# ZhangXiaze/DeepPointMap

Hardware: AMD Instinct MI355X
Metric: LiDAR frames/s (encode+match+register), 65 536 pts/frame (higher is better)
Workload: dtype f32 (attention scores K Q^T and P V, Linear / Conv1d (+ LayerNorm) layers with K <= 2048 as exact three-way bf16 splits: 6 bf16 products per fp32 product, fp32 accumulate -- fp32 accuracy, bf16 matrix pipe; all else fp32); 1 GPU; synthetic 64x65536-pt scans per GPU: Encoder.forward + consecutive-frame registration_forward (256x256) + information matrix per frame; points_per_frame=65536, parallelism=frame-sharded x1, one RCCL gather of descriptors+edges per step, weights=procedural (deeppointmap_amd/weights.py), allocator_reserve_gib=16, geometry_waits_for_caller_stream=True

## Files before the change

deeppointmap_amd/_lib.py:

```python
from __future__ import annotations

import ctypes
import os

import torch
from ctypes import c_char_p, c_double, c_int, c_longlong, c_size_t, c_uint, c_void_p

_HERE = os.path.dirname(os.path.abspath(__file__))
LIB_PATH = os.environ.get("DPM_LIB") or os.path.join(_HERE, "libdpm_hip.so")
VERSION_EXPERIMENT = 0x40000000

P, I, D, LL = c_void_p, c_int, c_double, c_longlong

SIGNATURES = {
    "dpm_version": (I, []),
    "dpm_error_string": (c_char_p, [I]),
    "dpm_prepare_points": (I, [P, P, I, I, I, P, P, P]),
    "dpm_to_channel_first": (I, [P, I, I, I, P, P]),
    "dpm_to_channel_first_ld": (I, [P, I, I, I, P, I, P]),
    "dpm_emit_descriptors": (I, [P, P, P, I, I, I, D, P, P, P, P, P]),
    "dpm_nested_levels": (I, [P, P, I, I, I, P, P, P, P, P]),
    "dpm_gather_frames": (I, [P, LL, I, I, I, P, I, P, P]),
    "dpm_fps_workspace_bytes": (c_size_t, [I, I, I]),
    "dpm_fps": (I, [P, P, I, I, I, P, P, P, P, P]),
# ... 44 lines not shown
    "dpm_match_workspace_bytes": (c_size_t, [I, I, I, I]),
    "dpm_match_topk": (I, [P, P, I, I, I, I, D, I, P, P, P, P]),
    "dpm_pairing_workspace_bytes": (c_size_t, [I, I, I]),
    "dpm_dual_softmax_topk": (I, [P, I, I, I, D, I, P, P, P, P]),
    "dpm_gather_pairs": (I, [P, P, P, I, I, I, I, I, P, P, P, P]),
    "dpm_mean_rows": (I, [P, I, I, I, P, I, P]),
    "dpm_kabsch_workspace_bytes": (c_size_t, [I, I]),
    "dpm_corr_kabsch": (I, [P, P, I, LL, P, I, LL, P, P, P, I, I, D, I, D, P, P, P, I, P]),
    "dpm_preprocess_workspace_bytes": (c_size_t, [LL]),
    "dpm_preprocess_scan": (I, [P, I, I, D, D, D, D, LL, P, P, I, P, P, P]),
    "dpm_knn_self_workspace_bytes": (c_size_t, [I]),
    "dpm_knn_self": (I, [P, I, I, D, P, P, P, P, P]),
    "dpm_point_normals": (I, [P, I, D, P, P, P]),
    "dpm_lowpass_similarity": (I, [P, P, I, I, I, P, P]),
    "dpm_stat_filter": (I, [P, I, D, I, D, P, P, P, P, P, P]),
    "dpm_filter_dc_workspace_bytes": (c_size_t, [I, I]),
    "dpm_outlier_filter_dc": (I, [P, P, P, I, I, D, D, D, P, P, P, P, P]),
    "dpm_lowpass_filter_dc": (I, [P, P, P, I, D, I, D, I, D, D, P, P, P, P, P]),
    "dpm_augment_workspace_bytes": (c_size_t, [I, LL]),
    "dpm_ground_filter": (I, [P, P, P, I, I, I, D, D, I, P, P, P, P, P]),
    "dpm_voxel_select": (I, [P, P, P, I, D, I, LL, P, P, P, P, P]),
    "dpm_mask_select": (I, [P, P, P, I, I, D, D, P, D, P, I, P, P, P, P, P]),
    "dpm_points_affine": (I, [P, P, I, I, P, P, P]),
    "dpm_points_deskew": (I, [P, P, P, I, I, P, I, I, P, D, P]),
    "dpm_gather_points": (I, [P, P, P, I, P, I, I, P, P, P, P]),
    "dpm_pack_frames": (I, [P, P, P, I, I, P, P, P, P]),
    "dpm_ingest_frames": (I, [P, P, LL, I, I, I, P, P, P, P, P]),
    "dpm_map_tile": (I, [P, P, P, P, I, I, I, P, P]),
    "dpm_infomat_workspace_bytes": (c_size_t, [I, I, I]),
    "dpm_information_matrix": (I, [P, I, P, I, P, D, P, P, P]),
    "dpm_information_matrix_batched": (I, [P, I, P, P, I, P, I, D, P, I, P, P]),
    "dpm_infomat_build_grids": (I, [P, I, P, I, D, P, P]),
    "dpm_infomat_search_grids": (I, [P, I, P, P, I, P, I, D, P, I, P, P]),
    "dpm_icp_workspace_bytes": (c_size_t, [I, I]),
    "dpm_icp_refine_batched": (I, [P, I, I, P, P, P, P, I, P, I, P, P, I, D, D, P, P, P, P, P, P, P, P, P]),
    "dpm_voxel_map_workspace_bytes": (c_size_t, [LL]),
    "dpm_voxel_map_init": (I, [LL, P, P]),
    "dpm_voxel_map_bounds": (I, [P, P, P, I, LL, P, P]),
    "dpm_voxel_map_insert": (I, [P, P, P, I, LL, LL, LL, D, D, D, D, P, P]),
    "dpm_voxel_map_finish": (I, [LL, P, P]),
    "dpm_voxel_map_emit": (I, [P, LL, D, D, D, D, P, P, I, P]),
    "dpm_reg_loss_pairs": (I, [P, P, I, I, I, D, P, P, P, P, P]),
    "dpm_reg_loss_workspace_bytes": (c_size_t, [I, I, I, I]),
    "dpm_reg_loss_forward": (I, [P, P, P, P, P, P, P, P, I, I, I, I, D, D, I, P, P, P, P, P, P]),
    "dpm_reg_loss_backward": (I, [P, P, P, P, I, I, I, I, D, D, I, P, P, P, P, P, P]),
    "dpm_attention_train_workspace_bytes": (c_size_t, [I, I, I, I]),
    "dpm_attention_train_forward": (I, [P, I, LL, P, I, LL, P, I, LL, P, I, LL, P, I, I, I, I, I, P, P]),
    "dpm_attention_train_backward": (I, [P, I, LL, P, I, LL, P, I, LL, P, I, LL, P, P, I, LL, P, P, P, P, I, I, I, I, I, P, P]),
    "dpm_offset_pairs_count": (I, [P, P, P, P, I, I, I, D, P, P, P]),
    "dpm_offset_pairs_fill": (I, [P, P, P, P, I, I, I, D, P, P, P]),
    "dpm_offset_pairs_gather": (I, [P, I, P, I, I, LL, I, P, P]),
    "dpm_offset_pairs_segment_sum": (I, [P, I, P, P, LL, I, P, P]),
    "dpm_group_train_forward": (I, [P, P, P, P, P, I, P, P, I, I, I, I, I, D, P, P, P]),
    "dpm_group_train_workspace_bytes": (c_size_t, [I, I, I, I, I]),
    "dpm_group_train_backward": (I, [P, P, P, P, P, I, P, I, I, I, I, I, D, P, P, P, P, P, P, P, P]),
    "dpm_loop_pool_workspace_bytes": (c_size_t, [I, I, I]),
    "dpm_loop_pool_forward": (I, [P, I, P, P, I, I, I, P, P, P]),
    "dpm_loop_pool_backward": (I, [P, I, P, P, P, I, I, I, P, P, P, P]),
    "dpm_loop_bce_forward": (I, [P, P, I, P, P, P, P]),
    "dpm_dense_train_workspace_bytes": (c_size_t, [LL, I, I]),
    "dpm_dense_train_forward": (I, [P, I, P, I, P, P, P, P, P, LL, I, I, I, P, P, P, P]),
    "dpm_dense_train_backward_rows": (I, [P, P, P, P, P, LL, I, I, P, P, P, P, P, P]),
    "dpm_dense_train_backward_gemm": (I, [P, P, I, P, I, LL, I, I, P, P, P, P, P]),
    "dpm_map_poses": (I, [P, P, P, P, P, I, I, I, P, P, P]),
    "dpm_map_assemble_fwd": (I, [P, P, P, P, P, I, I, I, I, I, D, P, P, P, P, P, P, P]),
    "dpm_map_assemble_bwd": (I, [P, P, I, I, I, I, I, P, P]),
# ... 93 lines not shown
```

deeppointmap_amd/csrc/infomat.hip:

```cpp
#include "block_scan.h"
#include "cell_grid.h"
#include "workspace.h"
#include <type_traits>

namespace {

constexpr int GMAX = 512;

struct PairArgs {
    const float *pcd1, *pcd2;
    const int32_t *f1, *f2;
    long long stride1, stride2;
    const float *Rt;
    int rt_stride;
    float *out;
    int out_stride;
    char *ws;
    size_t ws_stride;
    int N1, N2;
};

struct GridHdr {
    float lox, loy, inv_cs;
    int gx, gy, ncell;
    int H;
    int qexp;
};

__device__ __forceinline__ const float *pair_p1(const PairArgs &a, int p) {
    return a.pcd1 + (size_t)(a.f1 ? a.f1[p] : p) * a.stride1;
}
__device__ __forceinline__ const float *pair_p2(const PairArgs &a, int p) {
    return a.pcd2 + (size_t)(a.f2 ? a.f2[p] : p) * a.stride2;
}
__device__ __forceinline__ GridHdr *pair_hdr(const PairArgs &a, int p) { return (GridHdr *)(a.ws + (size_t)p * a.ws_stride); }
__device__ __forceinline__ int *pair_count(const PairArgs &a, int p) { return (int *)(a.ws + (size_t)p * a.ws_stride + 256); }
__device__ __forceinline__ float4 *pair_sorted(const PairArgs &a, int p) {
    return (float4 *)(a.ws + (size_t)p * a.ws_stride + 256 + sizeof(int) * (size_t)(GMAX * GMAX + 1) + 12);
}
__device__ __forceinline__ long long *pair_partial(const PairArgs &a, int p) {
    return (long long *)(pair_sorted(a, p) + a.N2);
}

constexpr int GB_CHUNK = 4096;

__device__ __forceinline__ float *pair_bounds(const PairArgs &a, int p);

__global__ __launch_bounds__(256) void grid_bounds_kernel(PairArgs A) {
    const int chunk = blockIdx.x, pair = blockIdx.y, chunks = gridDim.x;
    const float *p2 = pair_p2(A, pair);
    const int N2 = A.N2;
    __shared__ float red[5][4];
    const int t = threadIdx.x, lane = t & 63, w = t >> 6;
    float lox = __builtin_inff(), loy = lox, hix = -lox, hiy = -lox, amax = 0.f;
    constexpr int PPT = GB_CHUNK / 256;
    const int i0 = chunk * GB_CHUNK + t;
    float xs[PPT], ys[PPT], zs[PPT];
#pragma unroll
    for (int u = 0; u < PPT; ++u) {
        const int i = min(i0 + u * 256, N2 - 1);
        xs[u] = p2[i], ys[u] = p2[(size_t)N2 + i], zs[u] = p2[2 * (size_t)N2 + i];
    }
#pragma unroll
    for (int u = 0; u < PPT; ++u) {
        lox = fminf(lox, xs[u]), hix = fmaxf(hix, xs[u]), loy = fminf(loy, ys[u]), hiy = fmaxf(hiy, ys[u]);
        amax = fmaxf(amax, fmaxf(fmaxf(fabsf(xs[u]), fabsf(ys[u])), fabsf(zs[u])));
    }
#pragma unroll
    for (int off = 32; off > 0; off >>= 1) {
        lox = fminf(lox, __shfl_xor(lox, off, 64)), loy = fminf(loy, __shfl_xor(loy, off, 64));
        hix = fmaxf(hix, __shfl_xor(hix, off, 64)), hiy = fmaxf(hiy, __shfl_xor(hiy, off, 64));
        amax = fmaxf(amax, __shfl_xor(amax, off, 64));
// ... 144 lines not shown
#pragma unroll
    for (int u = 0; u < RB; ++u)
        if (lo + lane + u * 64 < hi) atomicAdd(&c[cell_coord(v[u].x, lox, inv_cs, gx)], 1);
    for (int p = lo + lane + RB * 64; p < hi; p += 64) atomicAdd(&c[cell_coord(tmp[p].x, lox, inv_cs, gx)], 1);
    __builtin_amdgcn_wave_barrier();
    const int per = (gx + 63) / 64, a = min(lane * per, gx), b = min(a + per, gx);
    int sum = 0;
    for (int k = a; k < b; ++k) sum += c[k];
    int run = lo + wave_scan_inclusive(sum) - sum;
    for (int k = a; k < b; ++k) {
        const int n = c[k];
        c[k] = run, run += n;
    }
    __builtin_amdgcn_wave_barrier();
    for (int k = lane; k < gx; k += 64) start[(size_t)row * gx + k] = c[k];
    if (row == gy - 1 && lane == 0) start[(size_t)gy * gx] = A.N2;
    __builtin_amdgcn_wave_barrier();
#pragma unroll
    for (int u = 0; u < RB; ++u)
        if (lo + lane + u * 64 < hi) sorted[atomicAdd(&c[cell_coord(v[u].x, lox, inv_cs, gx)], 1)] = v[u];
    for (int p = lo + lane + RB * 64; p < hi; p += 64) {
        const float4 q = tmp[p];
        sorted[atomicAdd(&c[cell_coord(q.x, lox, inv_cs, gx)], 1)] = q;
    }
}

__device__ __forceinline__ float quad_xor1(float v) { return __int_as_float(dpp_i<0xB1, 0xF>(__float_as_int(v))); }
__device__ __forceinline__ float quad_xor2(float v) { return __int_as_float(dpp_i<0x4E, 0xF>(__float_as_int(v))); }
__device__ __forceinline__ float quad_min(float v) {
    v = fminf(v, quad_xor1(v));
    return fminf(v, quad_xor2(v));
}

__global__ __launch_bounds__(256) void nn1_match_kernel(PairArgs A, float r2, int ordered) {
    int pair, blk;
    pair_block(blk, pair);
    const float *p1 = pair_p1(A, pair);
    const float *p2 = pair_p2(A, pair);
    const int N1 = A.N1, N2 = A.N2;
    const float *Rt = A.Rt + (size_t)pair * A.rt_stride;
    const GridHdr *hdr = pair_hdr(A, pair);
    const int *start = pair_count(A, pair);
    const float4 *sorted = pair_sorted(A, pair);
    __shared__ int s_qp;
    __shared__ long long sred[4][10];
    const int quad = threadIdx.x >> 2, ql = threadIdx.x & 3;
    if (threadIdx.x == 0) s_qp = -1;
    __syncthreads();
    if (ordered && A.f1 && A.f2 && N1 == N2)
        for (int t = threadIdx.x; t < (int)gridDim.y; t += 256)
            if (A.f2[t] == A.f1[pair]) atomicMax(&s_qp, t);
    __syncthreads();
    const float4 *qsorted = s_qp >= 0 ? pair_sorted(A, s_qp) : nullptr;
    const int gx = hdr->gx, gy = hdr->gy, H = hdr->H;
    const float inv_cs = hdr->inv_cs, cs = 1.0f / inv_cs, lox = hdr->lox, loy = hdr->loy;
    const float k2 = cs * cs * (1.f - 1e-5f);
    constexpr int NR = 5;
    int win[4] = {-1, -1, -1, -1};
    const int i_own = blk * 256 + ql * 64 + quad;
    float o_qx, o_qy, o_qz, o_below, o_above;
    int o_rlo[NR], o_rhi[NR];
    {
        const int ic = min(i_own, N1 - 1);
        float x, y, z;
        if (qsorted) {
            const float4 q4 = qsorted[ic];
            x = q4.x, y = q4.y, z = q4.z;
        } else {
            x = p1[ic], y = p1[(size_t)N1 + ic], z = p1[2 * (size_t)N1 + ic];
        }
        o_qx = fmaf(Rt[2], z, fmaf(Rt[1], y, Rt[0] * x)) + Rt[9];
        o_qy = fmaf(Rt[5], z, fmaf(Rt[4], y, Rt[3] * x)) + Rt[10];
        o_qz = fmaf(Rt[8], z, fmaf(Rt[7], y, Rt[6] * x)) + Rt[11];
        const float fx = (o_qx - lox) * inv_cs, fy = (o_qy - loy) * inv_cs;
        const float flx = floorf(fx), fly = floorf(fy);
        const int cx = (int)fmaxf(fminf(flx, 1e6f), -1e6f), cy = (int)fmaxf(fminf(fly, 1e6f), -1e6f);
        const int xa = min(max(cx - H, 0), gx), xb = min(max(cx + H + 1, 0), gx);
#pragma unroll
        for (int r = 0; r < NR; ++r) {
            const int k = (r + 1) / 2 * ((r & 1) ? -1 : 1);
            const int yy = cy + k;
            const bool in = yy >= 0 && yy < gy && (r < 3 || H > 1);
            const int yc = min(max(yy, 0), gy - 1);
            o_rlo[r] = in ? start[yc * gx + xa] : 0, o_rhi[r] = in ? start[yc * gx + xb] : 0;
        }
        o_below = fy - fly, o_above = fly + 1.f - fy;
    }
    auto one_query = [&](auto Jc) {
        constexpr int j = decltype(Jc)::value;
        constexpr int BC = j * 0x55;
        const int i = blk * 256 + j * 64 + quad;
        if (i >= N1) return;
        auto from_j = [&](int v) { return __builtin_amdgcn_update_dpp(v, v, BC, 0xF, 0xF, false); };
        auto from_jf = [&](float v) { return __int_as_float(from_j(__float_as_int(v))); };
        const float qx = from_jf(o_qx), qy = from_jf(o_qy), qz = from_jf(o_qz);
        int rlo[NR], rhi[NR];
#pragma unroll
        for (int r = 0; r < NR; ++r) rlo[r] = from_j(o_rlo[r]), rhi[r] = from_j(o_rhi[r]);
        const float mg = 1e-3f;
        unsigned long long best = ~0ull;
        auto offer = [&](const float4 t, bool ok) {
            const float dx = qx - t.x, dy = qy - t.y, dz = qz - t.z;
            const float d = (dx * dx + dy * dy) + dz * dz;
            const unsigned long long key = ((unsigned long long)__float_as_uint(d) << 32) | (unsigned)__float_as_int(t.w);
            best = (ok && key < best) ? key : best;
        };
        auto rest = [&](int from, int hi) {
            for (int p = from; p < hi; p += 8) {
                const float4 t0 = sorted[p], t1 = sorted[min(p + 4, hi - 1)];
                offer(t0, true), offer(t1, p + 4 < hi);
            }
        };
        {
            float4 t[3][2];
            bool ok[3][2];
#pragma unroll
            for (int r = 0; r < 3; ++r) {
#pragma unroll
                for (int u = 0; u < 2; ++u) {
                    const int p = rlo[r] + ql + 4 * u;
                    ok[r][u] = p < rhi[r];
                    t[r][u] = sorted[ok[r][u] ? p : 0];
                }
            }
#pragma unroll
            for (int r = 0; r < 3; ++r) offer(t[r][0], ok[r][0]), offer(t[r][1], ok[r][1]);
#pragma unroll
            for (int r = 0; r < 3; ++r) rest(rlo[r] + ql + 8, rhi[r]);
        }
        if (H > 1) {
            const float bd = best == ~0ull ? r2 : fminf(__uint_as_float((unsigned)(best >> 32)), r2);
            const float below = from_jf(o_below), above = from_jf(o_above);
            const float g0 = fmaxf(below + 1.f - mg, 0.f), g1 = fmaxf(above + 1.f - mg, 0.f);
            const int h3 = (g0 * g0 * k2 > bd) ? 0 : rhi[3], h4 = (g1 * g1 * k2 > bd) ? 0 : rhi[4];
            const int p3 = rlo[3] + ql, p4 = rlo[4] + ql;
            const float4 a0 = sorted[p3 < h3 ? p3 : 0], a1 = sorted[p3 + 4 < h3 ? p3 + 4 : 0];
            const float4 b0 = sorted[p4 < h4 ? p4 : 0], b1 = sorted[p4 + 4 < h4 ? p4 + 4 : 0];
            offer(a0, p3 < h3), offer(a1, p3 + 4 < h3), offer(b0, p4 < h4), offer(b1, p4 + 4 < h4);
            rest(p3 + 8, h3), rest(p4 + 8, h4);
        }
#pragma unroll
        for (int step = 0; step < 2; ++step) {
            const float blo = __int_as_float((int)(unsigned)best), bhi = __int_as_float((int)(unsigned)(best >> 32));
            const unsigned olo = (unsigned)__float_as_int(step ? quad_xor2(blo) : quad_xor1(blo));
            const unsigned ohi = (unsigned)__float_as_int(step ? quad_xor2(bhi) : quad_xor1(bhi));
            const unsigned long long o = ((unsigned long long)ohi << 32) | olo;
            best = o < best ? o : best;
        }
        win[j] = (best != ~0ull && __uint_as_float((unsigned)(best >> 32)) <= r2) ? (int)(unsigned)best : -1;
    };
    one_query(std::integral_constant<int, 0>{});
    one_query(std::integral_constant<int, 1>{});
    one_query(std::integral_constant<int, 2>{});
    one_query(std::integral_constant<int, 3>{});
    long long m[10] = {0, 0, 0, 0, 0, 0, 0, 0, 0, 0};
    if (ql == 0) {
        const float qs = ldexpf(1.f, hdr->qexp);
        float X[4], Y[4], Z[4];
#pragma unroll
        for (int j = 0; j < 4; ++j) {
            const int oi = max(win[j], 0);
            X[j] = p2[oi], Y[j] = p2[(size_t)N2 + oi], Z[j] = p2[2 * (size_t)N2 + oi];
        }
#pragma unroll
        for (int j = 0; j < 4; ++j) {
            if (win[j] < 0) continue;
            const long long x = (long long)__float2int_rn(X[j] * qs), y = (long long)__float2int_rn(Y[j] * qs),
                            z = (long long)__float2int_rn(Z[j] * qs);
            m[0] += 1, m[1] += x, m[2] += y, m[3] += z, m[4] += x * x, m[5] += y * y, m[6] += z * z;
            m[7] += x * y, m[8] += x * z, m[9] += y * z;
        }
    }
    const int lane = threadIdx.x & 63, w = threadIdx.x >> 6;
#pragma unroll
    for (int k = 0; k < 10; ++k) {
        long long v = m[k];
#pragma unroll
        for (int off = 32; off > 0; off >>= 1) v += __shfl_xor(v, off, 64);
        if (lane == 0) sred[w][k] = v;
    }
    __syncthreads();
    if (threadIdx.x < 10)
        pair_partial(A, pair)[(size_t)blk * 10 + threadIdx.x] =
            (sred[0][threadIdx.x] + sred[1][threadIdx.x]) + (sred[2][threadIdx.x] + sred[3][threadIdx.x]);
}

__global__ __launch_bounds__(64) void infomat_finalize_kernel(PairArgs A) {
    const long long *part = pair_partial(A, blockIdx.x);
    const int nblk = (A.N1 + 255) / 256, lane = threadIdx.x;
    __shared__ long long s[10];
    for (int k = 0; k < 10; ++k) {
        long long v = 0;
        for (int b = lane; b < nblk; b += 64) v += part[(size_t)b * 10 + k];
        v = wave_sum(v);
        if (lane == 0) s[k] = v;
    }
    __syncthreads();
    if (lane != 0) return;
    float *out = A.out + (size_t)blockIdx.x * A.out_stride;
    const int qexp = pair_hdr(A, blockIdx.x)->qexp;
    const double u = ldexp(1.0, -qexp), u2 = ldexp(1.0, -2 * qexp);
    const double n = (double)s[0], x = (double)s[1] * u, y = (double)s[2] * u, z = (double)s[3] * u, xx = (double)s[4] * u2,
                 yy = (double)s[5] * u2, zz = (double)s[6] * u2, xy = (double)s[7] * u2, xz = (double)s[8] * u2,
                 yz = (double)s[9] * u2;
    const double G[36] = {zz + yy, -xy,     -xz,     0,  -z, y,
                          -xy,     zz + xx, -yz,     z,  0,  -x,
                          -xz,     -yz,     yy + xx, -y, x,  0,
                          0,       z,       -y,      n,  0,  0,
                          -z,      0,       x,       0,  n,  0,
                          y,       -x,      0,       0,  0,  n};
    for (int i = 0; i < 36; ++i) out[i] = (float)G[i];
}

}

static size_t ws_slice_bytes(int N1, int N2) {
    size_t b = 256 + sizeof(int) * (size_t)(GMAX * GMAX + 1) + 12 + sizeof(float4) * (size_t)N2 +
               10 * sizeof(long long) * (size_t)dpm_cdiv(N1, 256) +
               sizeof(float4) * (size_t)N2 + sizeof(int) * ((size_t)dpm_cdiv(N2, GB_CHUNK) * (GMAX + 8) + GMAX + 4);
    return ws_align256(b);
}

extern "C" size_t dpm_infomat_workspace_bytes(int n_pairs, int N1, int N2) {
    return 256 + (size_t)n_pairs * ws_slice_bytes(N1, N2);
}

static int launch_grid(PairArgs A, int n_pairs, double radius, hipStream_t st) {
    const int fine = dpm_knob("DPM_NN1_FINE", 1);
    const int chunks = dpm_cdiv(A.N2, GB_CHUNK);
    hipLaunchKernelGGL(grid_bounds_kernel, dim3(chunks, n_pairs), dim3(256), 0, st, A);
    hipLaunchKernelGGL(grid_setup_kernel, dim3(n_pairs), dim3(64), 0, st, A, (float)radius, fine, chunks);
    if (dpm_knob("DPM_ABLATE_GRID", 0)) return dpm_launch_status();
    hipLaunchKernelGGL(grid_rows_kernel<false>, dim3(chunks, n_pairs), dim3(256), 0, st, A);
    hipLaunchKernelGGL(grid_offsets_kernel, dim3(n_pairs), dim3(256), 0, st, A);
    hipLaunchKernelGGL(grid_rows_kernel<true>, dim3(chunks, n_pairs), dim3(256), 0, st, A);
    hipLaunchKernelGGL(grid_cells_kernel, dim3(GMAX / 4, n_pairs), dim3(256), 0, st, A);
    return dpm_launch_status();
}

static int launch_search(PairArgs A, int n_pairs, double radius, hipStream_t st) {
    if (dpm_knob("DPM_ABLATE_NN1", 0)) return DPM_OK;
    const int ord = dpm_knob("DPM_NN1_ORDERED", 1);
    hipLaunchKernelGGL(nn1_match_kernel, dim3(dpm_cdiv(A.N1, 256), n_pairs), dim3(256), 0, st, A,
                       (float)(radius * radius), ord);
    hipLaunchKernelGGL(infomat_finalize_kernel, dim3(n_pairs), dim3(64), 0, st, A);
    return dpm_launch_status();
}

static int launch_infomat(PairArgs A, int n_pairs, double radius, hipStream_t st) {
    const int rc = launch_grid(A, n_pairs, radius, st);
    return rc ? rc : launch_search(A, n_pairs, radius, st);
}

static PairArgs batched_args(const float *pcd, int N, const int32_t *src_frame, const int32_t *dst_frame,
                             void *workspace) {
    PairArgs A{};
    A.pcd1 = pcd, A.pcd2 = pcd, A.f1 = src_frame, A.f2 = dst_frame, A.stride1 = 3LL * N, A.stride2 = 3LL * N;
    A.ws = (char *)ws_align256((uintptr_t)workspace), A.ws_stride = ws_slice_bytes(N, N);
    A.N1 = N, A.N2 = N;
    return A;
}

extern "C" int dpm_information_matrix(const float *pcd1, int N1, const float *pcd2, int N2, const float *Rt,
                                      double radius, float *out6x6, void *workspace, dpm_stream_t stream) {
    DPM_CHECK_ARG(pcd1 && pcd2 && Rt && out6x6 && workspace && N1 >= 1 && N2 >= 1 && radius > 0.0);
    PairArgs A{};
    A.pcd1 = pcd1, A.pcd2 = pcd2, A.f1 = nullptr, A.f2 = nullptr, A.stride1 = 0, A.stride2 = 0;
    A.Rt = Rt, A.rt_stride = 0, A.out = out6x6, A.out_stride = 0;
    A.ws = (char *)ws_align256((uintptr_t)workspace), A.ws_stride = ws_slice_bytes(N1, N2);
    A.N1 = N1, A.N2 = N2;
    return launch_infomat(A, 1, radius, (hipStream_t)stream);
}

extern "C" int dpm_information_matrix_batched(const float *pcd, int N, const int32_t *src_frame,
                                              const int32_t *dst_frame, int n_pairs, const float *Rt, int rt_stride,
                                              double radius, float *out, int out_stride, void *workspace,
                                              dpm_stream_t stream) {
    DPM_CHECK_ARG(pcd && src_frame && dst_frame && Rt && out && workspace && N >= 1 && n_pairs >= 1 && radius > 0.0);
    DPM_CHECK_ARG(rt_stride >= 12 && out_stride >= 36);
    PairArgs A = batched_args(pcd, N, src_frame, dst_frame, workspace);
    A.Rt = Rt, A.rt_stride = rt_stride, A.out = out, A.out_stride = out_stride;
    return launch_infomat(A, n_pairs, radius, (hipStream_t)stream);
}

extern "C" int dpm_infomat_build_grids(const float *pcd, int N, const int32_t *dst_frame, int n_pairs, double radius,
                                       void *workspace, dpm_stream_t stream) {
    DPM_CHECK_ARG(pcd && dst_frame && workspace && N >= 1 && n_pairs >= 1 && radius > 0.0);
    return launch_grid(batched_args(pcd, N, nullptr, dst_frame, workspace), n_pairs, radius, (hipStream_t)stream);
}

extern "C" int dpm_infomat_search_grids(const float *pcd, int N, const int32_t *src_frame, const int32_t *dst_frame,
                                        int n_pairs, const float *Rt, int rt_stride, double radius, float *out,
                                        int out_stride, void *workspace, dpm_stream_t stream) {
    DPM_CHECK_ARG(pcd && src_frame && dst_frame && Rt && out && workspace && N >= 1 && n_pairs >= 1 && radius > 0.0);
    DPM_CHECK_ARG(rt_stride >= 12 && out_stride >= 36);
    PairArgs A = batched_args(pcd, N, src_frame, dst_frame, workspace);
    A.Rt = Rt, A.rt_stride = rt_stride, A.out = out, A.out_stride = out_stride;
    return launch_search(A, n_pairs, radius, (hipStream_t)stream);
}
```

deeppointmap_amd/ops.py:

```python
from __future__ import annotations

from typing import Optional, Tuple

import ctypes
import threading
import weakref

import torch

from . import _lib, knobs

ACT_NONE, ACT_RELU, ACT_SIGMOID = 0, 1, 2


def _ptr(t: Optional[torch.Tensor]):
    return None if t is None else t.data_ptr()


def _stream(t: torch.Tensor):
    return torch.cuda.current_stream(t.device).cuda_stream


def _chk(t: torch.Tensor, dtype, name: str):
    if not t.is_cuda:
# ... 775 lines not shown
    _rows2d(out, "out")
    B, R, C = x.shape
    _lib.check(_lib.load().dpm_mean_rows(_ptr(x), B, R, C, _ptr(out), out.stride(0), _stream(x)), "dpm_mean_rows")


RES_HDR = 20


def corr_kabsch(offsets, src_xyz, dst_xyz, src_idx, dst_idx, conf, eps_offset: float, num_iter: int = 3,
                std_ratio: float = 3.0, header_out: Optional[torch.Tensor] = None, batch: int = 1) -> torch.Tensor:
    _chk(conf, torch.float32, "conf")
    _rows2d(src_xyz, "src_xyz"), _rows2d(dst_xyz, "dst_xyz")
    k = conf.shape[-1]
    if offsets is not None:
        _chk(offsets, torch.float32, "offsets")
        _chk(src_idx, torch.int32, "src_idx"), _chk(dst_idx, torch.int32, "dst_idx")
    lib = _lib.load()
    ws = torch.empty(lib.dpm_kabsch_workspace_bytes(batch, k), device=conf.device, dtype=torch.uint8)
    result = torch.empty(batch, RES_HDR + 2 * k, device=conf.device, dtype=torch.float32)
    hs = 0
    if header_out is not None:
        if header_out.dim() == 1:
            header_out = header_out.unsqueeze(0)
        _rows2d(header_out, "header_out")
        hs = header_out.stride(0)
    Ms, Md = src_xyz.shape[0] // batch, dst_xyz.shape[0] // batch
    _lib.check(lib.dpm_corr_kabsch(_ptr(offsets), _ptr(src_xyz), src_xyz.stride(0), Ms * src_xyz.stride(0),
                                   _ptr(dst_xyz), dst_xyz.stride(0), Md * dst_xyz.stride(0), _ptr(src_idx),
                                   _ptr(dst_idx), _ptr(conf), batch, k, float(eps_offset), num_iter, float(std_ratio),
                                   _ptr(ws), _ptr(result), _ptr(header_out), hs, _stream(conf)), "dpm_corr_kabsch")
    return result[0] if (batch == 1 and conf.dim() == 1) else result


def information_matrix(pcd1: torch.Tensor, pcd2: torch.Tensor, Rt: torch.Tensor, radius: float = 1.0,
                       out: Optional[torch.Tensor] = None) -> torch.Tensor:
    _chk(pcd1, torch.float32, "pcd1"), _chk(pcd2, torch.float32, "pcd2"), _chk(Rt, torch.float32, "Rt")
    N1, N2 = pcd1.shape[1], pcd2.shape[1]
    lib = _lib.load()
    ws = torch.empty(lib.dpm_infomat_workspace_bytes(1, N1, N2), device=pcd1.device, dtype=torch.uint8)
    if out is None:
        out = torch.empty(6, 6, device=pcd1.device, dtype=torch.float32)
    else:
        _chk(out, torch.float32, "out")
    _lib.check(lib.dpm_information_matrix(_ptr(pcd1), N1, _ptr(pcd2), N2, _ptr(Rt), float(radius), _ptr(out),
                                          _ptr(ws), _stream(pcd1)), "dpm_information_matrix")
    return out


def information_matrix_batched(pcd: torch.Tensor, src_frame: torch.Tensor, dst_frame: torch.Tensor, Rt_rows: torch.Tensor,
                               out_rows: torch.Tensor, radius: float = 1.0, grids: Optional[torch.Tensor] = None) -> None:
    _chk(pcd, torch.float32, "pcd"), _chk(src_frame, torch.int32, "src_frame"), _chk(dst_frame, torch.int32, "dst_frame")
    _rows2d(Rt_rows, "Rt_rows"), _rows2d(out_rows, "out_rows")
    P_, N = src_frame.numel(), pcd.shape[2]
    lib = _lib.load()
    if grids is not None:
        if grids.numel() != lib.dpm_infomat_workspace_bytes(P_, N, N):
            raise ValueError("grids was built for a different (n_pairs, N)")
        _lib.check(lib.dpm_infomat_search_grids(_ptr(pcd), N, _ptr(src_frame), _ptr(dst_frame), P_, _ptr(Rt_rows),
                                                Rt_rows.stride(0), float(radius), _ptr(out_rows), out_rows.stride(0),
                                                _ptr(grids), _stream(pcd)), "dpm_infomat_search_grids")
        return
    ws = torch.empty(lib.dpm_infomat_workspace_bytes(P_, N, N), device=pcd.device, dtype=torch.uint8)
    _lib.check(lib.dpm_information_matrix_batched(_ptr(pcd), N, _ptr(src_frame), _ptr(dst_frame), P_, _ptr(Rt_rows),
                                                  Rt_rows.stride(0), float(radius), _ptr(out_rows), out_rows.stride(0),
                                                  _ptr(ws), _stream(pcd)), "dpm_information_matrix_batched")


def information_matrix_grids(pcd: torch.Tensor, dst_frame: torch.Tensor, radius: float = 1.0) -> torch.Tensor:
    _chk(pcd, torch.float32, "pcd"), _chk(dst_frame, torch.int32, "dst_frame")
    P_, N = dst_frame.numel(), pcd.shape[2]
    lib = _lib.load()
    ws = torch.empty(lib.dpm_infomat_workspace_bytes(P_, N, N), device=pcd.device, dtype=torch.uint8)
    _lib.check(lib.dpm_infomat_build_grids(_ptr(pcd), N, _ptr(dst_frame), P_, float(radius), _ptr(ws), _stream(pcd)),
               "dpm_infomat_build_grids")
    return ws


ICP_POINT, ICP_PLANE = 0, 1
ICP_CONVERGED, ICP_MAX_ITER, ICP_NO_MATCH, ICP_SINGULAR = 0, 1, 2, 3
ICP_NSUM = 29


def icp_target_normals(pcd: torch.Tensor, lengths: torch.Tensor, dst_frame: torch.Tensor, radius: float = 1.0, host=None,
                       out: Optional[torch.Tensor] = None) -> torch.Tensor:
    _chk(pcd, torch.float32, "pcd"), _chk(lengths, torch.int32, "lengths"), _chk(dst_frame, torch.int32, "dst_frame")
    F, _, N = pcd.shape
    lib = _lib.load()
    normals = torch.zeros(F, N, 3, device=pcd.device, dtype=torch.float32) if out is None else _chk(out, torch.float32, "out")
    if tuple(normals.shape) != (F, N, 3):
        raise ValueError("out: expected (F,N,3)")
    ws = torch.empty(lib.dpm_knn_self_workspace_bytes(N), device=pcd.device, dtype=torch.uint8)
    frames, counts = (dst_frame.tolist(), lengths.tolist()) if host is None else host
    for f in sorted(set(int(f) for f in frames)):
        if not 0 <= f < F:
            raise ValueError(f"dst_frame: frame {f} outside [0, {F})")
        n = min(max(int(counts[f]), 0), N)
        if n == 0:
            continue
# ... 1641 lines not shown
```

include/dpm_hip.h:

```cpp
#ifndef DPM_HIP_H
#define DPM_HIP_H

#include <stddef.h>
#include <stdint.h>

#ifdef __cplusplus
extern "C" {
#endif

typedef void *dpm_stream_t;

#define DPM_OK 0
#define DPM_EINVAL (-1)
#define DPM_EUNSUPPORTED (-2)

#define DPM_ACT_NONE 0
#define DPM_ACT_RELU 1
#define DPM_ACT_SIGMOID 2

#define DPM_VERSION_EXPERIMENT 0x40000000
int dpm_version(void);
const char *dpm_error_string(int status);

int dpm_prepare_points(const float *points_cf, const uint8_t *padding, int B, int C, int N,
// ... 210 lines not shown
int dpm_mask_select(const float *xyz, const int32_t *idx_in, const int32_t *count, int capacity, int use_distance,
                    double min_dis, double max_dis, const float *u, double drop_ratio, const float *wedges, int n_wedges,
                    float *out_xyz, int32_t *out_idx, int32_t *out_count, void *workspace, dpm_stream_t stream);
int dpm_points_affine(float *xyz, const int32_t *count, int capacity, int mode, const double *params,
                      const float *jitter, dpm_stream_t stream);
int dpm_gather_points(const float *xyz, const int32_t *idx_in, const int32_t *count, int capacity, const int32_t *sel,
                      int n_sel, int limit, float *out_xyz, int32_t *out_idx, int32_t *out_count, dpm_stream_t stream);
int dpm_points_deskew(float *xyz, const int32_t *idx, const int32_t *count, int capacity, int time_mode, const float *times,
                      int n_times, int azimuth_steps, const double *motion, double s_ref, dpm_stream_t stream);
int dpm_pack_frames(const float *const *xyz, const int32_t *const *counts, const int32_t *capacities, int S,
                    int padding_to, float *points, unsigned char *padding, int32_t *status, dpm_stream_t stream);


int dpm_ingest_frames(const void *staging_host, void *staging_dev, long long staging_bytes, int F, int capacity,
                      int chunk, float *xyz, int32_t *idx, int32_t *count, void *workspace, dpm_stream_t stream);


int dpm_map_tile(const float *key_points, const int32_t *select, const float *poses, const float *centering,
                 int C, int S, int K, float *out, dpm_stream_t stream);


size_t dpm_infomat_workspace_bytes(int n_pairs, int N1, int N2);
int dpm_information_matrix(const float *pcd1, int N1, const float *pcd2, int N2, const float *Rt,
                           double radius, float *out6x6, void *workspace, dpm_stream_t stream);
int dpm_information_matrix_batched(const float *pcd, int N, const int32_t *src_frame,
                                   const int32_t *dst_frame, int n_pairs, const float *Rt, int rt_stride,
                                   double radius, float *out, int out_stride, void *workspace,
                                   dpm_stream_t stream);
int dpm_infomat_build_grids(const float *pcd, int N, const int32_t *dst_frame, int n_pairs, double radius,
                            void *workspace, dpm_stream_t stream);
int dpm_infomat_search_grids(const float *pcd, int N, const int32_t *src_frame, const int32_t *dst_frame,
                             int n_pairs, const float *Rt, int rt_stride, double radius, float *out,
                             int out_stride, void *workspace, dpm_stream_t stream);


#define DPM_ICP_POINT 0
#define DPM_ICP_PLANE 1
#define DPM_ICP_CONVERGED 0
#define DPM_ICP_MAX_ITER 1
#define DPM_ICP_NO_MATCH 2
#define DPM_ICP_SINGULAR 3
size_t dpm_icp_workspace_bytes(int n_pairs, int N);
int dpm_icp_refine_batched(const float *pcd, int F, int N, const int32_t *lengths, const float *normals,
                           const int32_t *src_frame, const int32_t *dst_frame, int n_pairs, const double *init_pose,
                           int metric, const double *stage_max_dist, const int32_t *stage_max_iter, int n_stages,
                           double tol_rot, double tol_trans, double *pose, float *fitness, float *rmse,
                           int32_t *iterations, int32_t *status, int32_t *debug_match, double *debug_system,
                           void *workspace, dpm_stream_t stream);


size_t dpm_voxel_map_workspace_bytes(long long n_points);
int dpm_voxel_map_init(long long n_points, void *workspace, dpm_stream_t stream);
int dpm_voxel_map_bounds(const float *const *clouds, const long long *offsets, const float *poses, int n_scans,
                         long long n_batch, void *workspace, dpm_stream_t stream);
int dpm_voxel_map_insert(const float *const *clouds, const long long *offsets, const float *poses, int n_scans,
                         long long n_batch, long long base, long long n_points, double min_x, double min_y,
                         double min_z, double voxel_size, void *workspace, dpm_stream_t stream);
int dpm_voxel_map_finish(long long n_points, void *workspace, dpm_stream_t stream);
int dpm_voxel_map_emit(const void *workspace, long long n_points, double min_x, double min_y, double min_z,
                       double voxel_size, float *centroids, int32_t *counts, int M, dpm_stream_t stream);

int dpm_reg_loss_pairs(const float *xyz_a, const float *xyz_b, int B, int M, int N, double eps, int32_t *nn_a, int32_t *nn_b,
                       int32_t *neutral_a, int32_t *neutral_b, dpm_stream_t stream);
size_t dpm_reg_loss_workspace_bytes(int B, int M, int N, int C);
int dpm_reg_loss_forward(const float *fea_a, const float *fea_b, const float *xyz_a, const float *xyz_b, const uint8_t *pad_a,
                         const uint8_t *pad_b, const int32_t *nn_a, const int32_t *nn_b, int B, int M, int N, int C, double tau,
// ... 207 lines not shown
```

Measured before the change: 16730 frames/s.

## Stage nearest-neighbour candidate cells into LDS tile for infomat matching

```diff
diff --git a/deeppointmap_amd/_lib.py b/deeppointmap_amd/_lib.py
--- a/deeppointmap_amd/_lib.py
+++ b/deeppointmap_amd/_lib.py
@@ -100,6 +100,7 @@
     "dpm_information_matrix_batched": (I, [P, I, P, P, I, P, I, D, P, I, P, P]),
     "dpm_infomat_build_grids": (I, [P, I, P, I, D, P, P]),
     "dpm_infomat_search_grids": (I, [P, I, P, P, I, P, I, D, P, I, P, P]),
+    "dpm_infomat_tile_blocks": (I, [P, I, I, I, P, P]),
     "dpm_icp_workspace_bytes": (c_size_t, [I, I]),
     "dpm_icp_refine_batched": (I, [P, I, I, P, P, P, P, I, P, I, P, P, I, D, D, P, P, P, P, P, P, P, P, P]),
     "dpm_voxel_map_workspace_bytes": (c_size_t, [LL]),
diff --git a/deeppointmap_amd/csrc/infomat.hip b/deeppointmap_amd/csrc/infomat.hip
--- a/deeppointmap_amd/csrc/infomat.hip
+++ b/deeppointmap_amd/csrc/infomat.hip
@@ -1,11 +1,14 @@
 #include "block_scan.h"
 #include "cell_grid.h"
 #include "workspace.h"
+#include <climits>
 #include <type_traits>
 
 namespace {
 
 constexpr int GMAX = 512;
+constexpr int R_MAX = 12, T_MAX = 2432, WG_BLOCKS = 2, NN1_THREADS = 256 * WG_BLOCKS;
+constexpr int COPY_U = 2;
 
 struct PairArgs {
     const float *pcd1, *pcd2;
@@ -25,6 +28,7 @@
     int gx, gy, ncell;
     int H;
     int qexp;
+    int tile_blocks;
 };
 
 __device__ __forceinline__ const float *pair_p1(const PairArgs &a, int p) {
@@ -38,6 +42,7 @@
 __device__ __forceinline__ float4 *pair_sorted(const PairArgs &a, int p) {
     return (float4 *)(a.ws + (size_t)p * a.ws_stride + 256 + sizeof(int) * (size_t)(GMAX * GMAX + 1) + 12);
 }
+constexpr long long TILE_FLAG = 1ll << 32;
 __device__ __forceinline__ long long *pair_partial(const PairArgs &a, int p) {
     return (long long *)(pair_sorted(a, p) + a.N2);
 }
@@ -248,9 +253,11 @@
     return fminf(v, quad_xor2(v));
 }
 
-__global__ __launch_bounds__(256) void nn1_match_kernel(PairArgs A, float r2, int ordered) {
-    int pair, blk;
-    pair_block(blk, pair);
+__global__ __launch_bounds__(NN1_THREADS, 8) void nn1_match_kernel(
+PairArgs A, float r2, int ordered) {
+    int pair, wg;
+    pair_block(wg, pair);
+    const int part = threadIdx.x >> 8, tid = threadIdx.x & 255, blk = wg * WG_BLOCKS + part;
     const float *p1 = pair_p1(A, pair);
     const float *p2 = pair_p2(A, pair);
     const int N1 = A.N1, N2 = A.N2;
@@ -259,12 +266,17 @@
     const int *start = pair_count(A, pair);
     const float4 *sorted = pair_sorted(A, pair);
     __shared__ int s_qp;
-    __shared__ long long sred[4][10];
-    const int quad = threadIdx.x >> 2, ql = threadIdx.x & 3;
-    if (threadIdx.x == 0) s_qp = -1;
+    __shared__ long long sred[WG_BLOCKS][4][10];
+    __shared__ int s_c0, s_c1;
+    __shared__ int s_qlo[R_MAX + 4], s_qhi[R_MAX + 4];
+    __shared__ int s_rowg[R_MAX], s_rowl[R_MAX + 1];
+    __shared__ float4 s_tile[T_MAX];
+    const int quad = tid >> 2, ql = tid & 3;
+    if (threadIdx.x == 0) s_qp = -1, s_c0 = INT_MAX, s_c1 = INT_MIN;
+    if (threadIdx.x < R_MAX + 4) s_qlo[threadIdx.x] = INT_MAX, s_qhi[threadIdx.x] = 0;
     __syncthreads();
     if (ordered && A.f1 && A.f2 && N1 == N2)
-        for (int t = threadIdx.x; t < (int)gridDim.y; t += 256)
+        for (int t = threadIdx.x; t < (int)gridDim.y; t += NN1_THREADS)
             if (A.f2[t] == A.f1[pair]) atomicMax(&s_qp, t);
     __syncthreads();
     const float4 *qsorted = s_qp >= 0 ? pair_sorted(A, s_qp) : nullptr;
@@ -276,6 +288,7 @@
     const int i_own = blk * 256 + ql * 64 + quad;
     float o_qx, o_qy, o_qz, o_below, o_above;
     int o_rlo[NR], o_rhi[NR];
+    int o_cy, o_xa, o_xb;
     {
         const int ic = min(i_own, N1 - 1);
         float x, y, z;
@@ -301,9 +314,68 @@
             o_rlo[r] = in ? start[yc * gx + xa] : 0, o_rhi[r] = in ? start[yc * gx + xb] : 0;
         }
         o_below = fy - fly, o_above = fly + 1.f - fy;
-    }
-    auto one_query = [&](auto Jc) {
+        o_cy = cy, o_xa = xa, o_xb = xb;
+    }
+    bool tile = false;
+    {
+        const bool asks = i_own < N1 && o_xa < o_xb && o_cy + H >= 0 && o_cy - H <= gy - 1;
+        const int cmin = wave_min_dpp(asks ? o_cy : INT_MAX), cmax = -wave_min_dpp(asks ? -o_cy : INT_MAX);
+        if ((threadIdx.x & 63) == 0 && cmin != INT_MAX) atomicMin(&s_c0, cmin), atomicMax(&s_c1, cmax);
+        __syncthreads();
+        const int c0 = __builtin_amdgcn_readfirstlane(s_c0), c1 = __builtin_amdgcn_readfirstlane(s_c1);
+        const int y0 = c0 <= c1 ? max(c0 - H, 0) : 0, rows = c0 <= c1 ? min(c1 + H, gy - 1) - y0 + 1 : 0;
+        if (rows <= R_MAX) {
+            if (asks) atomicMin(&s_qlo[o_cy - c0], o_xa), atomicMax(&s_qhi[o_cy - c0], o_xb);
+            __syncthreads();
+            if (threadIdx.x < 64) {
+                const int k = threadIdx.x, y = y0 + k;
+                int lo = INT_MAX, hi = 0, g = 0, len = 0;
+                if (k < rows) {
+                    for (int c = max(y - H, c0); c <= min(y + H, c1); ++c) lo = min(lo, s_qlo[c - c0]), hi = max(hi, s_qhi[c - c0]);
+                    if (lo < hi) g = start[y * gx + lo], len = start[y * gx + hi] - g;
+                }
+                const int end = wave_scan_inclusive(len);
+                if (k < rows) s_rowg[k] = g, s_rowl[k] = end - len;
+                if (k == 63) s_rowl[rows] = end;
+            }
+            __syncthreads();
+            const int total = __builtin_amdgcn_readfirstlane(s_rowl[rows]);
+            if (total <= T_MAX) {
+                tile = true;
+                int k = 0;
+                for (int t0 = threadIdx.x; t0 < total; t0 += COPY_U * NN1_THREADS) {
+                    int from[COPY_U];
+#pragma unroll
+                    for (int u = 0; u < COPY_U; ++u) {
+                        const int t = min(t0 + u * NN1_THREADS, total - 1);
+                        while (t >= s_rowl[k + 1]) ++k;
+                        from[u] = s_rowg[k] + (t - s_rowl[k]);
+                    }
+                    float4 v[COPY_U];
+#pragma unroll
+                    for (int u = 0; u < COPY_U; ++u) v[u] = sorted[from[u]];
+#pragma unroll
+                    for (int u = 0; u < COPY_U; ++u)
+                        if (t0 + u * NN1_THREADS < total) s_tile[t0 + u * NN1_THREADS] = v[u];
+                }
+#pragma unroll
+                for (int r = 0; r < NR; ++r) {
+                    const int yy = o_cy + (r + 1) / 2 * ((r & 1) ? -1 : 1);
+                    const bool in = asks && yy >= 0 && yy < gy && (r < 3 || H > 1);
+                    const int kk = in ? yy - y0 : 0, shift = s_rowl[kk] - s_rowg[kk];
+                    o_rlo[r] = in ? o_rlo[r] + shift : 0, o_rhi[r] = in ? o_rhi[r] + shift : 0;
+                }
+                __syncthreads();
+            }
+        }
+    }
+    auto one_query = [&](auto Jc, auto Tc) {
         constexpr int j = decltype(Jc)::value;
+        constexpr bool TILE = decltype(Tc)::value;
+        auto cand = [&](int p) -> float4 {
+            if constexpr (TILE) return s_tile[p];
+            else return sorted[p];
+        };
         constexpr int BC = j * 0x55;
         const int i = blk * 256 + j * 64 + quad;
         if (i >= N1) return;
@@ -323,7 +395,7 @@
         };
         auto rest = [&](int from, int hi) {
             for (int p = from; p < hi; p += 8) {
-                const float4 t0 = sorted[p], t1 = sorted[min(p + 4, hi - 1)];
+                const float4 t0 = cand(p), t1 = cand(min(p + 4, hi - 1));
                 offer(t0, true), offer(t1, p + 4 < hi);
             }
         };
@@ -336,7 +408,7 @@
                 for (int u = 0; u < 2; ++u) {
                     const int p = rlo[r] + ql + 4 * u;
                     ok[r][u] = p < rhi[r];
-                    t[r][u] = sorted[ok[r][u] ? p : 0];
+                    t[r][u] = cand(ok[r][u] ? p : 0);
                 }
             }
 #pragma unroll
@@ -350,8 +422,8 @@
             const float g0 = fmaxf(below + 1.f - mg, 0.f), g1 = fmaxf(above + 1.f - mg, 0.f);
             const int h3 = (g0 * g0 * k2 > bd) ? 0 : rhi[3], h4 = (g1 * g1 * k2 > bd) ? 0 : rhi[4];
             const int p3 = rlo[3] + ql, p4 = rlo[4] + ql;
-            const float4 a0 = sorted[p3 < h3 ? p3 : 0], a1 = sorted[p3 + 4 < h3 ? p3 + 4 : 0];
-            const float4 b0 = sorted[p4 < h4 ? p4 : 0], b1 = sorted[p4 + 4 < h4 ? p4 + 4 : 0];
+            const float4 a0 = cand(p3 < h3 ? p3 : 0), a1 = cand(p3 + 4 < h3 ? p3 + 4 : 0);
+            const float4 b0 = cand(p4 < h4 ? p4 : 0), b1 = cand(p4 + 4 < h4 ? p4 + 4 : 0);
             offer(a0, p3 < h3), offer(a1, p3 + 4 < h3), offer(b0, p4 < h4), offer(b1, p4 + 4 < h4);
             rest(p3 + 8, h3), rest(p4 + 8, h4);
         }
@@ -365,10 +437,14 @@
         }
         win[j] = (best != ~0ull && __uint_as_float((unsigned)(best >> 32)) <= r2) ? (int)(unsigned)best : -1;
     };
-    one_query(std::integral_constant<int, 0>{});
-    one_query(std::integral_constant<int, 1>{});
-    one_query(std::integral_constant<int, 2>{});
-    one_query(std::integral_constant<int, 3>{});
+    auto four_queries = [&](auto Tc) {
+        one_query(std::integral_constant<int, 0>{}, Tc);
+        one_query(std::integral_constant<int, 1>{}, Tc);
+        one_query(std::integral_constant<int, 2>{}, Tc);
+        one_query(std::integral_constant<int, 3>{}, Tc);
+    };
+    if (tile) four_queries(std::true_type{});
+    else four_queries(std::false_type{});
     long long m[10] = {0, 0, 0, 0, 0, 0, 0, 0, 0, 0};
     if (ql == 0) {
         const float qs = ldexpf(1.f, hdr->qexp);
@@ -387,18 +463,20 @@
             m[7] += x * y, m[8] += x * z, m[9] += y * z;
         }
     }
-    const int lane = threadIdx.x & 63, w = threadIdx.x >> 6;
+    const bool has_blk = blk * 256 < N1;
+    if (tid == 0 && tile && has_blk) m[0] += TILE_FLAG;
+    const int lane = tid & 63, w = tid >> 6;
 #pragma unroll
     for (int k = 0; k < 10; ++k) {
         long long v = m[k];
 #pragma unroll
         for (int off = 32; off > 0; off >>= 1) v += __shfl_xor(v, off, 64);
-        if (lane == 0) sred[w][k] = v;
+        if (lane == 0) sred[part][w][k] = v;
     }
     __syncthreads();
-    if (threadIdx.x < 10)
-        pair_partial(A, pair)[(size_t)blk * 10 + threadIdx.x] =
-            (sred[0][threadIdx.x] + sred[1][threadIdx.x]) + (sred[2][threadIdx.x] + sred[3][threadIdx.x]);
+    if (tid < 10 && has_blk)
+        pair_partial(A, pair)[(size_t)blk * 10 + tid] =
+            (sred[part][0][tid] + sred[part][1][tid]) + (sred[part][2][tid] + sred[part][3][tid]);
 }
 
 __global__ __launch_bounds__(64) void infomat_finalize_kernel(PairArgs A) {
@@ -414,9 +492,11 @@
     __syncthreads();
     if (lane != 0) return;
     float *out = A.out + (size_t)blockIdx.x * A.out_stride;
-    const int qexp = pair_hdr(A, blockIdx.x)->qexp;
+    GridHdr *hdr = pair_hdr(A, blockIdx.x);
+    const int qexp = hdr->qexp;
+    hdr->tile_blocks = (int)(s[0] / TILE_FLAG);
     const double u = ldexp(1.0, -qexp), u2 = ldexp(1.0, -2 * qexp);
-    const double n = (double)s[0], x = (double)s[1] * u, y = (double)s[2] * u, z = (double)s[3] * u, xx = (double)s[4] * u2,
+    const double n = (double)(s[0] % TILE_FLAG), x = (double)s[1] * u, y = (double)s[2] * u, z = (double)s[3] * u, xx = (double)s[4] * u2,
                  yy = (double)s[5] * u2, zz = (double)s[6] * u2, xy = (double)s[7] * u2, xz = (double)s[8] * u2,
                  yz = (double)s[9] * u2;
     const double G[36] = {zz + yy, -xy,     -xz,     0,  -z, y,
@@ -426,6 +506,11 @@
                           -z,      0,       x,       0,  n,  0,
                           y,       -x,      0,       0,  0,  n};
     for (int i = 0; i < 36; ++i) out[i] = (float)G[i];
+}
+
+__global__ __launch_bounds__(64) void tile_blocks_kernel(PairArgs A, int n_pairs, int32_t *counts) {
+    const int p = blockIdx.x * 64 + threadIdx.x;
+    if (p < n_pairs) counts[p] = pair_hdr(A, p)->tile_blocks;
 }
 
 }
@@ -457,7 +542,7 @@
 static int launch_search(PairArgs A, int n_pairs, double radius, hipStream_t st) {
     if (dpm_knob("DPM_ABLATE_NN1", 0)) return DPM_OK;
     const int ord = dpm_knob("DPM_NN1_ORDERED", 1);
-    hipLaunchKernelGGL(nn1_match_kernel, dim3(dpm_cdiv(A.N1, 256), n_pairs), dim3(256), 0, st, A,
+    hipLaunchKernelGGL(nn1_match_kernel, dim3(dpm_cdiv(A.N1, 256 * WG_BLOCKS), n_pairs), dim3(NN1_THREADS), 0, st, A,
                        (float)(radius * radius), ord);
     hipLaunchKernelGGL(infomat_finalize_kernel, dim3(n_pairs), dim3(64), 0, st, A);
     return dpm_launch_status();
@@ -514,3 +599,13 @@
     A.Rt = Rt, A.rt_stride = rt_stride, A.out = out, A.out_stride = out_stride;
     return launch_search(A, n_pairs, radius, (hipStream_t)stream);
 }
+
+extern "C" int dpm_infomat_tile_blocks(const void *workspace, int n_pairs, int N1, int N2, int32_t *counts,
+                                       dpm_stream_t stream) {
+    DPM_CHECK_ARG(workspace && counts && n_pairs >= 1 && N1 >= 1 && N2 >= 1);
+    PairArgs A{};
+    A.ws = (char *)ws_align256((uintptr_t)workspace), A.ws_stride = ws_slice_bytes(N1, N2);
+    A.N1 = N1, A.N2 = N2;
+    hipLaunchKernelGGL(tile_blocks_kernel, dim3(dpm_cdiv(n_pairs, 64)), dim3(64), 0, (hipStream_t)stream, A, n_pairs, counts);
+    return dpm_launch_status();
+}
diff --git a/deeppointmap_amd/ops.py b/deeppointmap_amd/ops.py
--- a/deeppointmap_amd/ops.py
+++ b/deeppointmap_amd/ops.py
@@ -831,8 +831,25 @@
     return result[0] if (batch == 1 and conf.dim() == 1) else result
 
 
+def information_matrix_tile_blocks(workspace: torch.Tensor, n_pairs: int, N1: int, N2: Optional[int] = None,
+                                   out: Optional[torch.Tensor] = None) -> torch.Tensor:
+    N2 = N1 if N2 is None else N2
+    lib = _lib.load()
+    if workspace.numel() != lib.dpm_infomat_workspace_bytes(n_pairs, N1, N2):
+        raise ValueError("workspace was sized for a different (n_pairs, N1, N2)")
+    if out is None:
+        out = torch.empty(n_pairs, device=workspace.device, dtype=torch.int32)
+    else:
+        _chk(out, torch.int32, "tile_blocks")
+        if out.numel() < n_pairs:
+            raise ValueError("tile_blocks holds fewer than n_pairs counts")
+    _lib.check(lib.dpm_infomat_tile_blocks(_ptr(workspace), n_pairs, N1, N2, _ptr(out), _stream(workspace)),
+               "dpm_infomat_tile_blocks")
+    return out
+
+
 def information_matrix(pcd1: torch.Tensor, pcd2: torch.Tensor, Rt: torch.Tensor, radius: float = 1.0,
-                       out: Optional[torch.Tensor] = None) -> torch.Tensor:
+                       out: Optional[torch.Tensor] = None, tile_blocks: Optional[torch.Tensor] = None) -> torch.Tensor:
     _chk(pcd1, torch.float32, "pcd1"), _chk(pcd2, torch.float32, "pcd2"), _chk(Rt, torch.float32, "Rt")
     N1, N2 = pcd1.shape[1], pcd2.shape[1]
     lib = _lib.load()
@@ -843,11 +860,14 @@
         _chk(out, torch.float32, "out")
     _lib.check(lib.dpm_information_matrix(_ptr(pcd1), N1, _ptr(pcd2), N2, _ptr(Rt), float(radius), _ptr(out),
                                           _ptr(ws), _stream(pcd1)), "dpm_information_matrix")
+    if tile_blocks is not None:
+        information_matrix_tile_blocks(ws, 1, N1, N2, out=tile_blocks)
     return out
 
 
 def information_matrix_batched(pcd: torch.Tensor, src_frame: torch.Tensor, dst_frame: torch.Tensor, Rt_rows: torch.Tensor,
-                               out_rows: torch.Tensor, radius: float = 1.0, grids: Optional[torch.Tensor] = None) -> None:
+                               out_rows: torch.Tensor, radius: float = 1.0, grids: Optional[torch.Tensor] = None,
+                               tile_blocks: Optional[torch.Tensor] = None) -> None:
     _chk(pcd, torch.float32, "pcd"), _chk(src_frame, torch.int32, "src_frame"), _chk(dst_frame, torch.int32, "dst_frame")
     _rows2d(Rt_rows, "Rt_rows"), _rows2d(out_rows, "out_rows")
     P_, N = src_frame.numel(), pcd.shape[2]
@@ -858,11 +878,15 @@
         _lib.check(lib.dpm_infomat_search_grids(_ptr(pcd), N, _ptr(src_frame), _ptr(dst_frame), P_, _ptr(Rt_rows),
                                                 Rt_rows.stride(0), float(radius), _ptr(out_rows), out_rows.stride(0),
                                                 _ptr(grids), _stream(pcd)), "dpm_infomat_search_grids")
+        if tile_blocks is not None:
+            information_matrix_tile_blocks(grids, P_, N, out=tile_blocks)
         return
     ws = torch.empty(lib.dpm_infomat_workspace_bytes(P_, N, N), device=pcd.device, dtype=torch.uint8)
     _lib.check(lib.dpm_information_matrix_batched(_ptr(pcd), N, _ptr(src_frame), _ptr(dst_frame), P_, _ptr(Rt_rows),
                                                   Rt_rows.stride(0), float(radius), _ptr(out_rows), out_rows.stride(0),
                                                   _ptr(ws), _stream(pcd)), "dpm_information_matrix_batched")
+    if tile_blocks is not None:
+        information_matrix_tile_blocks(ws, P_, N, out=tile_blocks)
 
 
 def information_matrix_grids(pcd: torch.Tensor, dst_frame: torch.Tensor, radius: float = 1.0) -> torch.Tensor:
diff --git a/include/dpm_hip.h b/include/dpm_hip.h
--- a/include/dpm_hip.h
+++ b/include/dpm_hip.h
@@ -266,6 +266,7 @@
 int dpm_infomat_search_grids(const float *pcd, int N, const int32_t *src_frame, const int32_t *dst_frame,
                              int n_pairs, const float *Rt, int rt_stride, double radius, float *out,
                              int out_stride, void *workspace, dpm_stream_t stream);
+int dpm_infomat_tile_blocks(const void *workspace, int n_pairs, int N1, int N2, int32_t *counts, dpm_stream_t stream);
 
 
 #define DPM_ICP_POINT 0
```

Result: no change. 16600 frames/s (-0.8%).
